# MarcoMeter/endless-memory-gym

Hardware: AMD Instinct MI355X
Metric: env steps/sec (aggregate) (higher is better)
Workload: dtype u8; 1 GPU; MortarMayhem-Grid-v0, 65536 envs/GPU x 1 GPU, 84x84x3 obs (u8_xyc), same-step auto-reset, uniform random actions generated on device; env_id=MortarMayhem-Grid-v0, envs_per_gpu=65536, envs_total=65536, parallelism=env-sharded x1, no data-path collective

## Files before the change

### endless-memory-gym_amd/csrc/mg_mortar.hip

```cpp
#include <memory>

#include "mg_atlas_v1.hpp"
#include "mg_lab.hpp"
#include "mg_option_sets.hpp"
#include "mg_stamps.hpp"
#include "mg_mortar_types.hpp"
#include "mg_mortar_compose.hpp"
#include "mg_raster_gather_v1.hpp"
#include "mg_mortar_step.hpp"
#include "mg_mortar_one_launch.hpp"
#include "mg_mortar_expert.hpp"
#include "mg_mortar_advance.hpp"
#include "mg_mortar_play.hpp"
#include "mg_mortar_trace.hpp"
#include "mg_mortar_next.hpp"

namespace mg {
using namespace v1;

__global__ __launch_bounds__(256) void mortar_init_kernel(int n, MortarState* state) {
    int i = blockIdx.x * blockDim.x + threadIdx.x;
    if (i >= n) return;
    MortarState s;
    memset(&s, 0, sizeof(s));
    s.disp_sprite = 0xFF;
    state[i] = s;
}

__global__ __launch_bounds__(256) void mortar_gt64_kernel(int n, const MortarState* state, double* out) {
    const int i = blockIdx.x * blockDim.x + threadIdx.x;
    if (i >= n) return;
    const MortarState s = state[i];
    out[2 * i] = s.tx / 5.0;
    out[2 * i + 1] = s.ty / 5.0;
}

__global__ __launch_bounds__(256) void mortar_gt64_masked_kernel(int n, const MortarState* state, double* out, const uint8_t* __restrict__ only) {
    const int i = blockIdx.x * blockDim.x + threadIdx.x;
    if (i >= n || !only[i]) return;
    const MortarState s = state[i];
    out[2 * i] = s.tx / 5.0;
    out[2 * i + 1] = s.ty / 5.0;
}

__global__ __launch_bounds__(256) void mortar_debug_desc_kernel(MortarParams P0, int n, MortarIO io, MortarDesc* out) {
    const int i = blockIdx.x * blockDim.x + threadIdx.x;
    if (i >= n) return;
    const MortarParams& P = io.set_of ? io.sets[set_index(io.set_of, i)] : P0;
    const MortarState s = io.state[i];
    const uint8_t* cmds = io.cmds + (size_t)i * P.cmd_cap;
    MortarDesc d = io.desc[i];
    {
        const bool have = s.disp_sprite != 0xFF;
        const int cx = (have && !s.disp_is_agent) ? s.disp_x : s.ax, cy = (have && !s.disp_is_agent) ? s.disp_y : s.ay;
        d.sx = (int16_t)(cx - P.sprite_dim / 2);
        d.sy = (int16_t)(cy - P.sprite_dim / 2);
        d.sprite = have ? s.disp_sprite : (uint8_t)0;
        d.tmpl = (uint16_t)((s.tiles_on && P.visual_feedback) ? 1 + s.tx * P.N + s.ty : 0);
        d.glyph_x0 = (int16_t)P.glyph_x0;
    }
    d.glyph = 0xFF;
    if (s.vis_pos < s.vis_len) {
        const int idx = (int)s.dbg_pops, period = s.show_dur + s.show_delay;
        io.state[i].dbg_pops = s.dbg_pops + 1;
        if (idx >= 0 && idx < (int)s.vis_len && period > 0) {
            const int k = idx / period, w = idx % period;
            d.glyph = (w < s.show_dur) ? cmds[s.vis_base + k] : (uint8_t)9;
        }
    }
    const int r = P.tile / 2;
    d.ring_x = (int16_t)(P.arena_x0 + P.tile * s.tx + P.tile / 2 - r);
    d.ring_y = (int16_t)(P.arena_x0 + P.tile * s.ty + P.tile / 2 - r);
    d.ring_on = 1;
    out[i] = d;
}

__device__ __forceinline__ MortarDesc mortar_debug_desc_one(const MortarParams& P, const MortarIO& io, int i) {
    const MortarState s = io.state[i];
    const uint8_t* cmds = io.cmds + (size_t)i * P.cmd_cap;
    MortarDesc d = io.desc[i];
    {
        const bool have = s.disp_sprite != 0xFF;
        const int cx = (have && !s.disp_is_agent) ? s.disp_x : s.ax, cy = (have && !s.disp_is_agent) ? s.disp_y : s.ay;
        d.sx = (int16_t)(cx - P.sprite_dim / 2);
        d.sy = (int16_t)(cy - P.sprite_dim / 2);
        d.sprite = have ? s.disp_sprite : (uint8_t)0;
        d.tmpl = (uint16_t)((s.tiles_on && P.visual_feedback) ? 1 + s.tx * P.N + s.ty : 0);
        d.glyph_x0 = (int16_t)P.glyph_x0;
    }
    d.glyph = 0xFF;
    if (s.vis_pos < s.vis_len) {
        const int idx = (int)s.dbg_pops, period = s.show_dur + s.show_delay;
        io.state[i].dbg_pops = s.dbg_pops + 1;
        if (idx >= 0 && idx < (int)s.vis_len && period > 0) {
            const int k = idx / period, w = idx % period;
            d.glyph = (w < s.show_dur) ? cmds[s.vis_base + k] : (uint8_t)9;
        }
    }
    const int r = P.tile / 2;
    d.ring_x = (int16_t)(P.arena_x0 + P.tile * s.tx + P.tile / 2 - r);
    d.ring_y = (int16_t)(P.arena_x0 + P.tile * s.ty + P.tile / 2 - r);
    d.ring_on = 1;
    return d;
}
__global__ __launch_bounds__(256) void mortar_debug_desc_picked_kernel(MortarParams P0, int n, MortarIO io, const int32_t* __restrict__ idx, int count,
                                                                       MortarDesc* rec) {
    const int j = blockIdx.x * blockDim.x + threadIdx.x;
    if (j >= count) return;
    const int i = idx ? idx[j] : j;
    if (i < 0) return;
    if (i >= n) return raise_error(io.err, ERR_FRAME_INDEX);
    const MortarParams& P = io.set_of ? io.sets[set_index(io.set_of, i)] : P0;
    rec[j] = mortar_debug_desc_one(P, io, i);
}

static const double SCALE = 0.25;

class MortarFamily : public Family {
   public:
    MortarFamily(int variant_id, int n) : Family(n), P_(sets_[0].P) {
        memset(&P_, 0, sizeof(P_));
        const int variant = variant_id >= 3 ? variant_id - 3 : variant_id;
        P_.variant = variant;
        P_.taskb = variant_id >= 3;
        agent_scale_ = 1.0 * SCALE;
        agent_speed_ = 12.0 * SCALE;
        P_.N = variant == V_ENDLESS ? 6 : 5;
        P_.allowed = variant == V_GRID ? 5 : 9;
        P_.visual_feedback = 1;
        P_.max_steps = -1;
        P_.initial_count = 1;
        P_.cmd_cap = variant == V_ENDLESS ? 512 : 32;
        if (variant == V_ENDLESS) {
            const int cap = lab_int("MEMGYM_EMM_CMD_CAP", 0);
            if (cap >= 4 && cap <= 512) P_.cmd_cap = cap;
        }
        MortarOpt& O = sets_[0];
        O.st_command_count.set(P_.command_count, {10});
        O.st_show_dur.set(P_.show_dur, {3});
        O.st_show_delay.set(P_.show_delay, {1});
        O.st_expl_dur.set(P_.expl_dur, {variant == V_GRID ? 2 : 6});
        O.st_expl_delay.set(P_.expl_delay, {variant == V_GRID ? 6 : 18});
        P_.r_fail = 0.0;
        P_.r_succ = 0.1;
        P_.r_ep_succ = 0.0;
        P_.r_new = 0.0;
        state_.alloc(n);
        cmds_.alloc((size_t)n * P_.cmd_cap);
        desc_.alloc(n);
        tdesc_.alloc(n);
        rng_.alloc(n);
        err_.alloc();
        claims_.alloc((size_t)((n + 255) / 256) * 4);
        handover_.alloc(n);
        rescues_.alloc(1);
        sets_.alloc();
        launch(mortar_init_kernel, dim3((n + 255) / 256), dim3(256), 0, 0, n, state_.p);
        MG_HIP(hipDeviceSynchronize());
        rebuild();
        sets_.defaults = P_;
    }

    void set_capacity(const std::string& what, int64_t v) override {
        if (!(P_.variant == V_ENDLESS && what == "commands")) return Family::set_capacity(what, v);
        if (v < 4 || v > 32768) throw OptionError{-3, "commands: 4 .. 32,768"};
        if (seeded_) throw std::runtime_error("mg_set_capacity: before the first reset");
        if (2 * P_.initial_count > v) throw OptionError{-3, "commands: below twice the initial_command_count in force"};
        MG_HIP(hipDeviceSynchronize());
        P_.cmd_cap = (int)v;
        cmds_.alloc((size_t)n_ * P_.cmd_cap);
        ++geom_gen_;
        sets_.refresh_geometry();
    }
    int64_t capacity(const std::string& what) const override {
        if (P_.variant == V_ENDLESS && what == "commands") return P_.cmd_cap;
        return Family::capacity(what);
    }
    void want_done_flag(uint32_t* flag_dev, uint32_t ticket) override {
        flag_dev_ = flag_dev;
        flag_ticket_ = ticket;
    }
    bool done_flag_stored() override {
        const bool stored = flag_stored_;
        flag_stored_ = false;
        return stored;
    }
    int action_dim() const override { return P_.variant == V_GRID ? 1 : 2; }
    int gt_dim() const override { return P_.variant == V_ENDLESS ? 2 : 0; }
    int vec_dim() const override { return P_.taskb ? VEC_DIM : 0; }
    void bind_vector_obs(float* dev) override {
        if (dev != vec_) ++geom_gen_;
        vec_ = dev;
    }
    const char* info_name(int k) const override {
        if (P_.variant == V_ENDLESS) return k == 0 ? "commands_completed" : (k == 1 ? "max_command_sequence" : nullptr);
        return k == 0 ? "success" : (k == 1 ? "commands_completed" : nullptr);
    }

    void set_option(const std::string& key, const double* v, int n) override { set_option_set(0, key, v, n); }
    void set_option_set(int set, const std::string& key, const double* v, int n) override {
        MortarOpt& O = sets_.ensure(set);
        MortarParams& P = O.P;
        const bool endless = P_.variant == V_ENDLESS;
        const OptionArg A{set, key, v, n, dirty_};
        if (key == "agent_scale") A.geometry(agent_scale_, v[0]);
        else if (key == "allowed_commands") {
            int a = A.integer();
            if (a < 4 || a > 9) throw OptionError{-4, "assert 4 <= allowed_commands <= 9"};
            P.allowed = a;
        }
        else if (!P_.taskb && key == "command_show_duration") O.st_show_dur.set(P.show_dur, A.int_list(1, 65535));
        else if (!P_.taskb && key == "command_show_delay") O.st_show_delay.set(P.show_delay, A.int_list(0, 65535));
        else if (key == "explosion_duration") O.st_expl_dur.set(P.expl_dur, A.int_list(1, 65535));
        else if (key == "explosion_delay") O.st_expl_delay.set(P.expl_delay, A.int_list(1, 65535));
        else if (key == "visual_feedback") P.visual_feedback = A.flag();
        else if (key == "reward_command_failure") P.r_fail = v[0];
        else if (key == "reward_command_success") P.r_succ = v[0];
        else if (endless && key == "max_steps") P.max_steps = A.integer();
        else if (endless && key == "initial_command_count") {
            int c = A.integer();
            if (c < 1 || c > P_.cmd_cap / 2) throw OptionError{-3, "initial_command_count out of the supported range"};
            P.initial_count = c;
        }
        else if (endless && key == "reward_new_command_success") P.r_new = v[0];
        else if (!endless && key == "arena_size") {
            int a = A.integer();
            if (a < 2 || a > MORTAR_MAX_N) throw OptionError{-4, "assert 2 <= arena_size <= 6"};
            if (a != P_.N) A.geometry(P_.N, a);
        }
        else if (!endless && key == "command_count") O.st_command_count.set(P.command_count, A.int_list(1, P_.taskb ? VEC_DIM / 9 : P_.cmd_cap));
        else if (!endless && key == "reward_episode_success") P.r_ep_succ = v[0];
        else if (P_.variant != V_GRID && key == "agent_speed") A.geometry(agent_speed_, v[0]);
        else throw OptionError{-2, "unknown reset parameter " + key};
    }
    void bind_option_sets(const int32_t* set_of_dev) override { sets_.bind(set_of_dev); }

    void reset(const int64_t* seeds, const uint8_t* mask, void* obs, float* gt, hipStream_t s) override {
        if (dirty_) rebuild();
        require_seeded(seeds);
        check_schedules();
        if (seeds) seeded_ = true;
        sets_.upload(s);
        with_bool(sets_.per_set(), [&](auto PS) {
            launch(mortar_reset_kernel<decltype(PS)::value>, dim3((n_ + 255) / 256), dim3(256), 0, s, P_, n_, io(), seeds, mask, gt_dim() ? gt : nullptr);
        });
        reset_frames(mask, [&](const uint8_t* m) { launch_raster_sparse<MortarComposer>(desc_.p, atlas_->dev(), obs, obs_format, n_, s, m); },
                     [&] { raster(obs, s); });
    }

    void step(const int32_t* actions, const uint8_t* active, void* obs, float* reward, uint8_t* done, float* gt, const mg_info_dev* info,
              int autoreset, hipStream_t s, void* final_frames) override {
        struct Consume {
            uint32_t*& flag;
            ~Consume() { flag = nullptr; }
        } consume{flag_dev_};
        flag_stored_ = false;
        const mg_info_dev ib = begin_step(info);
        sets_.upload(s);
        const MortarStepArgs sa = step_args(actions, reward, done, gt, ib, autoreset);
        if (obs && !active && one_launch(s)) {
            epoch_ = epoch_ % 255u + 1u;
            ++ticket_;
            const int logic_wgs = (n_ + 255) / 256;
            const int frames = frames_grid(n_);
            static const bool logic_last = lab_flag("MEMGYM_LAB_LOGIC_LAST", false);
            const bool store_flag = flag_dev_ && n_ == 1 && gt_dim() == 0 && obs_format == MG_OBS_U8_XYC;
            auto launch_step = [&](auto kernel, const MortarStepArgs& a, uint32_t* flag, uint32_t flag_ticket) {
                launch(kernel, dim3(logic_wgs + frames), dim3(256), RASTER_LDS, s, a, logic_wgs, logic_last ? frames : 0, epoch_, ticket_,
                               claims_.p, rescues_.p, atlas_->dev(), obs, flag, flag_ticket);
            };
            prof.begin(1, s);
            if (store_flag) {
                launch_step(mortar_step_raster_kernel<true>, sa, flag_dev_, flag_ticket_);
            } else if (ib.final_obs_dev && autoreset) {
                MortarStepArgs fa = sa;
                fa.tdesc = tdesc_.p;
                with_obs_format(obs_format, [&](auto F) { launch_step(mortar_step_raster_kernel<false, true, decltype(F)::value>, fa, nullptr, 0u); });
            } else {
                with_obs_format(obs_format, [&](auto F) { launch_step(mortar_step_raster_kernel<false, false, decltype(F)::value>, sa, nullptr, 0u); });
            }
            check_launch();
            ++one_launch_steps_;
            flag_stored_ = store_flag;
            prof.end(1, s);
            return;
        }
        prof.begin(0, s);
        const int sb = step_block(256);
        with_bool(sets_.per_set(), [&](auto PS) {
            if (final_frames) {
                with_bool(active != nullptr, [&](auto MASKED) {
                    launch(mortar_step_records_kernel<decltype(PS)::value, decltype(MASKED)::value>, dim3((n_ + sb - 1) / sb), dim3(sb), 0, s, sa, active,
                           (MortarDesc*)final_frames);
                });
            } else if (active) launch(mortar_step_masked_kernel<decltype(PS)::value>, dim3((n_ + sb - 1) / sb), dim3(sb), 0, s, sa, active);
            else launch(mortar_step_kernel<decltype(PS)::value>, dim3((n_ + sb - 1) / sb), dim3(sb), 0, s, sa);
        });
        end_logic(s);
        if (!obs) return;
        if (active) return masked_frames(obs, active, s);
        prof.begin(1, s);
        raster(obs, s);
        prof.end(1, s);
    }

    bool step_next(const int32_t* actions, const uint8_t* restart, uint8_t* restart_copy, void* obs, float* reward, uint8_t* done, float* gt,
                   const mg_info_dev* info, hipStream_t s) override {
        if (!lab_flag("MEMGYM_NEXT_FUSE", true)) return false;
        const mg_info_dev ib = begin_step(info);
        check_schedules();
        sets_.upload(s);
        const MortarStepArgs sa = step_args(actions, reward, done, gt, ib, 0);
        const int sb = step_block(256);
        prof.begin(0, s);
        with_bool(sets_.per_set(), [&](auto PS) {
            launch(mortar_step_next_kernel<decltype(PS)::value>, dim3((n_ + sb - 1) / sb), dim3(sb), 0, s, sa, restart, restart_copy);
        });
        end_logic(s);
        prof.begin(1, s);
        raster(obs, s);
        prof.end(1, s);
        with_bool(sets_.per_set(), [&](auto PS) {
            launch_checked(mortar_next_settle_kernel<decltype(PS)::value>, dim3((n_ + 255) / 256), dim3(256), 0, s, P_, n_, io(), (const uint8_t*)restart_copy);
        });
        return true;
    }

    bool advance(const AdvanceArgs& v, hipStream_t s) override {
        if (!lab_flag("MEMGYM_MORTAR_ADVANCE_FUSE", true)) return false;
        require_geometry();
        sets_.upload(s);
        const MortarStepArgs sa = step_args(v.actions, v.reward, v.done, v.gt, v.info, 1);
        rollout_chunks(v.steps, [&](int t0, int k) {
            with_bool(sets_.per_set(), [&](auto PS) {
                launch_checked(mortar_advance_kernel<decltype(PS)::value>, dim3((n_ + 255) / 256), dim3(256), 0, s, sa, advance_chunk(v, t0, k));
            });
        });
        return true;
    }
    bool play(const PlayArgs& v, hipStream_t s) override {
        if (!lab_flag("MEMGYM_MORTAR_PLAY_FUSE", true)) return false;
        require_geometry();
        sets_.upload(s);
        rollout_chunks(v.steps, [&](int t0, int k) {
            with_bool(sets_.per_set(), [&](auto PS) {
                launch_checked(mortar_play_kernel<decltype(PS)::value>, dim3((n_ + 255) / 256), dim3(256), 0, s, play_step_args(v, t0), play_chunk(v, t0, k));
            });
        });
        return true;
    }
    bool advance_traced(const AdvanceArgs& v, const TraceRows& tr, hipStream_t s) override {
        if (!lab_flag("MEMGYM_MORTAR_ADVANCE_FUSE", true)) return false;
        require_geometry();
        sets_.upload(s);
        const MortarStepArgs sa = step_args(v.actions, v.reward, v.done, v.gt, v.info, 1);
        const size_t row = (size_t)n_ * (size_t)action_dim();
        rollout_chunks(v.steps, [&](int t0, int k) {
            const MortarTraceRows rows{row_at((MortarDesc*)tr.frames, t0, n_), row_at(tr.actions, t0, row), row_at(tr.labels, t0, row), row_at(tr.reward, t0, n_),
                                       row_at(tr.done, t0, n_)};
            with_bool(sets_.per_set(), [&](auto PS) {
                launch_checked(mortar_advance_traced_kernel<decltype(PS)::value>, dim3((n_ + 255) / 256), dim3(256), 0, s, sa, advance_chunk(v, t0, k), rows);
            });
        });
        return true;
    }
    bool play_traced(const PlayArgs& v, void* frames, hipStream_t s) override {
        if (!lab_flag("MEMGYM_MORTAR_PLAY_FUSE", true)) return false;
        require_geometry();
        sets_.upload(s);
        rollout_chunks(v.steps, [&](int t0, int k) {
            with_bool(sets_.per_set(), [&](auto PS) {
                launch_checked(mortar_play_traced_kernel<decltype(PS)::value>, dim3((n_ + 255) / 256), dim3(256), 0, s, play_step_args(v, t0), play_chunk(v, t0, k),
                               row_at((MortarDesc*)frames, t0, n_));
            });
        });
        return true;
    }

    std::vector<std::pair<void*, size_t>> state_blobs() override {
        std::vector<std::pair<void*, size_t>> v = {{state_.p, state_.bytes()}, {cmds_.p, cmds_.bytes()}};
        rng_.blobs(v);
        return v;
    }

    std::vector<std::pair<void*, size_t>> instance_rows() override {
        std::vector<std::pair<void*, size_t>> v = {{state_.p, sizeof(MortarState)}, {cmds_.p, (size_t)P_.cmd_cap}, {desc_.p, sizeof(MortarDesc)}};
        rng_.rows(v);
        if (vec_) v.push_back({vec_, sizeof(float) * VEC_DIM});
        return v;
    }

    void expert_actions(const ExpertArgs& x, hipStream_t s) override {
        require_geometry();
        sets_.upload(s);
        launch_checked(mortar_expert_kernel, expert_grid(n_), dim3(EXPERT_BLOCK), 0, s, P_, n_, io(), x);
    }
    void ground_truth64(double* out, hipStream_t s, const uint8_t* only = nullptr) override {
        if (!gt_dim() || !out) return;
        if (only) return launch_checked(mortar_gt64_masked_kernel, dim3((n_ + 255) / 256), dim3(256), 0, s, n_, state_.p, out, only);
        launch_checked(mortar_gt64_kernel, dim3((n_ + 255) / 256), dim3(256), 0, s, n_, state_.p, out);
    }
    bool debug_counter(const std::string& name, int64_t* out) override {
        if (name == "cmd_list_max" || name == "cmd_list_ge12") {
            std::vector<MortarState> h(n_);
            MG_HIP(hipDeviceSynchronize());
            MG_HIP(hipMemcpy(h.data(), state_.p, sizeof(MortarState) * (size_t)n_, hipMemcpyDeviceToHost));
            int64_t mx = 0, ge = 0;
            for (const MortarState& s : h) {
                mx = s.num_cmds > mx ? s.num_cmds : mx;
                ge += s.num_cmds >= 12;
            }
            *out = name == "cmd_list_max" ? mx : ge;
            return true;
        }
        if (name == "one_launch_steps") {
            *out = one_launch_steps_;
            return true;
        }
        if (name != "one_launch_rescues") return false;
        uint32_t v = 0;
        MG_HIP(hipMemcpy(&v, rescues_.p, sizeof v, hipMemcpyDeviceToHost));
        *out = (int64_t)v;
        return true;
    }

    void raster_debug(void* frames, hipStream_t s) override {
        debug_frames<MortarDesc>(
            s, [&](MortarDesc* dbg) { launch(mortar_debug_desc_kernel, dim3((n_ + 255) / 256), dim3(256), 0, s, P_, n_, io(), dbg); },
            [&](MortarDesc* dbg) { launch_raster<MortarDebugComposer>(dbg, atlas_->dev(), frames, MG_OBS_U8_XYC, n_, s); });
    }

    void save_debug_records(const int32_t* idx, int count, void* rec, hipStream_t s) override {
        sets_.upload(s);
        launch_checked(mortar_debug_desc_picked_kernel, dim3((count + 255) / 256), dim3(256), 0, s, P_, n_, io(), idx, count, (MortarDesc*)rec);
    }
    void draw_debug_records(const void* records, int n_records, const int32_t* pick, int count, int size, void* rgb, hipStream_t s) override {
        launch_raster_debug_gather<MortarDebugComposer>((const MortarDesc*)records, atlas_->dev(), rgb, size, n_records, pick, count, err_.dev, s);
        check_launch();
    }

   private:
    uint32_t* flag_dev_ = nullptr;
    uint32_t flag_ticket_ = 0;
    bool flag_stored_ = false;
    int64_t one_launch_steps_ = 0;
    uint32_t ticket_ = 0;
    uint32_t epoch_ = 0;
    bool one_launch(hipStream_t s) { return fuse_step() && !sets_.per_set() && !stream_capturing(s); }
    static bool fuse_step() {
        static const bool on = lab_flag("MEMGYM_MORTAR_FUSE", true);
        return on;
    }
    void check_schedules() {
        for (size_t k = 0; k < sets_.size(); ++k) {
            const MortarOpt& O = sets_[k];
            const long long n_max = P_.variant == V_ENDLESS ? O.P.initial_count : O.st_command_count.max(O.P.command_count);
            if (!P_.taskb && n_max * ((long long)O.st_show_dur.max(O.P.show_dur) + O.st_show_delay.max(O.P.show_delay)) > 65535)
                throw OptionError{-3, "command_count x (command_show_duration + command_show_delay) exceeds the 65,535 entries of this build's display schedule"};
        }
    }
    MortarStepArgs step_args(const int32_t* actions, float* reward, uint8_t* done, float* gt, const mg_info_dev& ib, int autoreset) {
        return MortarStepArgs{P_, n_, io(), actions, reward, done, gt_dim() ? gt : nullptr, ib, autoreset, handover_.p, nullptr};
    }
    template <class F>
    static void rollout_chunks(int steps, F&& f) {
        for (int t0 = 0; t0 < steps; t0 += ADVANCE_MAX_STEPS) f(t0, steps - t0 < ADVANCE_MAX_STEPS ? steps - t0 : ADVANCE_MAX_STEPS);
    }
    template <class T>
    static T* row_at(T* base, int t0, size_t width) {
        return base ? base + (size_t)t0 * width : nullptr;
    }
    static MortarAdvanceArgs advance_chunk(const AdvanceArgs& v, int t0, int k) {
        return MortarAdvanceArgs{k, t0 == 0 ? 1 : 0, v.eps, v.seed, v.step0 + (uint64_t)t0, v.actions, v.out};
    }
    MortarStepArgs play_step_args(const PlayArgs& v, int t0) {
        return step_args(row_at(v.tape, t0, (size_t)n_ * (size_t)action_dim()), v.reward, v.done, v.gt, v.info, v.episode ? 0 : 1);
    }
    MortarPlayArgs play_chunk(const PlayArgs& v, int t0, int k) const {
        return MortarPlayArgs{k, t0 == 0 ? 1 : 0, t0 + k == v.steps ? 1 : 0, v.episode, n_ * action_dim(), v.active, v.alive, row_at(v.reward_trace, t0, n_),
                              row_at(v.done_trace, t0, n_), v.played, v.out};
    }
    MortarIO io() {
        MortarIO o;
        o.state = state_.p;
        o.cmds = cmds_.p;
        o.rng = rng_.view();
        o.desc = desc_.p;
        o.vec = vec_;
        o.err = err_.dev;
        o.sets = sets_.dev();
        o.set_of = sets_.set_of();
        return o;
    }

    void rebuild() {
        int radius = 0;
        std::vector<Stamp> sprites = build_agent_sprites(P_.variant == V_GRID ? 1.0 * SCALE : agent_scale_, &radius);
        std::vector<Stamp> glyphs = build_glyphs(SCALE);
        P_.tile = (int)(56 * SCALE);
        P_.arena_x0 = SCREEN / 2 - ((P_.tile * P_.N) >> 1);
        P_.radius = radius;
        P_.sprite_dim = sprites[0].w;
        double inv = 1.0 / std::sqrt(2.0);
        P_.v_axis = (1.0 / 1.0) * agent_speed_;
        P_.v_diag = inv * agent_speed_;
        P_.v_axis_i = (int)P_.v_axis;
        P_.v_diag_i = (int)P_.v_diag;
        P_.off_lo = (int)(-8 * SCALE);
        P_.off_hi = (int)(8 * SCALE);

        atlas_.reset(new Atlas());
        for (auto& sp : sprites) atlas_->add_stamp(sp);
        for (auto& g : glyphs) atlas_->add_stamp(g);
        {
            const int r = P_.tile / 2;
            Stamp ring_stamp(2 * r, 2 * r);
            circle(ring_stamp, r, r, r, (int)(8 * SCALE), 6);
            atlas_->add_stamp(ring_stamp);
        }
        atlas_->set_templates(build_mortar_templates(P_.N, SCALE, SCREEN));
        atlas_->upload();
        P_.glyph_x0 = (int)((SCREEN / 2) - std::floor(88 * SCALE / 2));
        dirty_ = false;
        ++geom_gen_;
        sets_.refresh_geometry();
    }

    struct MortarOpt {
        MortarParams P;
        OptListStore st_command_count, st_show_dur, st_show_delay, st_expl_dur, st_expl_delay;
        static void copy_geometry(MortarParams& d, const MortarParams& s) {
            d.variant = s.variant; d.N = s.N; d.taskb = s.taskb; d.cmd_cap = s.cmd_cap; d.arena_x0 = s.arena_x0; d.tile = s.tile;
            d.radius = s.radius; d.sprite_dim = s.sprite_dim; d.glyph_x0 = s.glyph_x0; d.v_axis_i = s.v_axis_i; d.v_diag_i = s.v_diag_i;
            d.off_lo = s.off_lo; d.off_hi = s.off_hi; d.v_axis = s.v_axis; d.v_diag = s.v_diag;
        }
    };

    void raster_only(void* obs, const uint8_t* only, hipStream_t s) override {
        launch_raster<MortarComposer>(desc_.p, atlas_->dev(), obs, obs_format, n_, s, only);
        check_launch();
    }
    std::pair<const void*, size_t> frame_rows() override { return {desc_.p, sizeof(MortarDesc)}; }
    void draw_records(const void* records, int n_records, const int32_t* pick, int count, int fmt, void* obs, hipStream_t s) override {
        launch_raster_gather<MortarComposer, false>((const MortarDesc*)records, atlas_->dev(), obs, fmt, n_records, pick, count, err_.dev, s);
        check_launch();
    }
    void draw_records_padded(const void* records, int n_records, const int32_t* pick, int count, int fmt, void* obs, hipStream_t s) override {
        launch_raster_gather<MortarComposer, true>((const MortarDesc*)records, atlas_->dev(), obs, fmt, n_records, pick, count, err_.dev, s);
        check_launch();
    }
    bool keeps_final_obs(hipStream_t s) override {
        static const bool wanted = lab_flag("MEMGYM_MORTAR_FINAL_FUSED", true);
        return wanted && one_launch(s);
    }

    void raster(void* obs, hipStream_t s) { raster_only(obs, nullptr, s); }

    OptionSets<MortarOpt> sets_;
    MortarParams& P_;
    std::unique_ptr<Atlas> atlas_;
    double agent_scale_, agent_speed_;
    float* vec_ = nullptr;
    DevArray<MortarState> state_;
    DevArray<uint8_t> cmds_;
    DevArray<MortarDesc> desc_;
    DevArray<uint32_t> claims_, rescues_;
    DevArray<uint64_t> handover_, tdesc_;
};

Family* make_mortar(int variant, int num_envs) { return new MortarFamily(variant, num_envs); }

}

#ifdef MG_LAB
extern "C" int mg_lab_set_window_offsets(const long long* off, int n) {
    long long v[16] = {0};
    for (int i = 0; i < n && i < 16; ++i) v[i] = off[i];
    return hipMemcpyToSymbol(HIP_SYMBOL(mg::v1::g_lab_win_off), v, sizeof v) == hipSuccess ? 0 : -1;
}
#endif
```

### endless-memory-gym_amd/csrc/mg_mortar_one_launch.hpp

```cpp
#pragma once
#include "mg_mortar_compose.hpp"
#include "mg_mortar_step.hpp"

namespace mg {
using namespace v1;

constexpr unsigned long long RESCUE_AFTER_TICKS = 20000;
__device__ __forceinline__ MortarDesc desc_from_handover(uint32_t lo, uint32_t hi, int glyph_x0) {
    const Handover f = unpack_handover(lo, hi);
    MortarDesc d;
    d.sx = (int16_t)f.sx, d.sy = (int16_t)f.sy, d.tmpl = (uint16_t)f.tmpl, d.sprite = (uint8_t)f.sprite, d.glyph = (uint8_t)f.glyph;
    d.glyph_x0 = (int16_t)glyph_x0;
    d.ring_x = d.ring_y = 0, d.ring_on = (uint8_t)f.ring_on, d.reserved = 0;
    return d;
}
constexpr int one_launch_wgs_per_cu(int fmt) { return fmt == MG_OBS_U8_XYC || fmt == MG_OBS_U8_CYX ? 7 : 6; }
template <bool DONE_FLAG, bool FINAL = false, int FMT = MG_OBS_U8_XYC>
__global__ __launch_bounds__(256, one_launch_wgs_per_cu(FMT)) void mortar_step_raster_kernel(MortarStepArgs a, int logic_wgs, int logic_base, uint32_t epoch,
                                                                    uint32_t ticket, uint32_t* claims, uint32_t* rescues,
                                                                    RasterAtlas A, void* __restrict__ obs, uint32_t* done_flag, uint32_t done_ticket) {
    constexpr bool ONE_BYTE = one_launch_wgs_per_cu(FMT) == 7;
    auto store = [](uint8_t* frame, void* dst, int env, int t) {
        if constexpr (ONE_BYTE) store_frame<FMT, false>(frame, dst, env, t);
        else store_frame<FMT, false, false, 1>(frame, dst, env, t & 255);
    };
    const int n = a.n;
    const int tid = threadIdx.x, lane = tid & 63;
    const int rel = (int)blockIdx.x - logic_base;
    const bool is_logic = rel >= 0 && rel < logic_wgs;
    auto claim = [&](int q) -> bool {
        uint32_t old = 0;
        if (lane == 0) old = __hip_atomic_exchange(claims + q, ticket, __ATOMIC_RELAXED, __HIP_MEMORY_SCOPE_AGENT);
        return (uint32_t)__builtin_amdgcn_readfirstlane((int)old) != ticket;
    };
    if (is_logic) {
        const int q = rel * 4 + (tid >> 6), i = q * 64 + lane;
#if defined(MG_LABV) && MG_LABV >= 1
        if (i < n) mortar_step_body<true, false, false, FINAL, DONE_FLAG>(i, a, epoch);
#else
        if (i < n) mortar_step_body<true, true, false, FINAL, DONE_FLAG>(i, a, epoch, claims + q, ticket);
#endif
        return;
    }
    extern __shared__ __attribute__((aligned(16))) uint8_t smem[];
    RasterCtx R = make_ctx(smem, A);
    const int stride = (int)gridDim.x - logic_wgs;
    for (int v = (int)blockIdx.x < logic_base ? (int)blockIdx.x : (int)blockIdx.x - logic_wgs; v < n; v += stride) {
        const int env = xcd_grouped_frame(v, n);
        const uint64_t* src = a.handover + env;
        uint32_t lo, hi;
        bool tried = false;
        unsigned long long t0 = 0;
        for (int polls = 0;; ++polls) {
            const uint64_t w = __hip_atomic_load(src, __ATOMIC_RELAXED, __HIP_MEMORY_SCOPE_AGENT);
            lo = (uint32_t)__builtin_amdgcn_readfirstlane((int)(uint32_t)w);
            hi = (uint32_t)__builtin_amdgcn_readfirstlane((int)(uint32_t)(w >> 32));
            if ((hi >> (HANDOVER_EPOCH_SHIFT - 32)) == epoch) break;
#if defined(MG_LABV) && MG_LABV >= 2
            if (false) {
#else
            if (polls == 0) t0 = wall_clock64();
            if (!tried && (polls & 15) == 15 && wall_clock64() - t0 >= RESCUE_AFTER_TICKS) {
#endif
                tried = true;
                if (claim(env >> 6)) {
                    const MortarStepArgs MG_KERNARG_AS* ka = kernarg_reread<MortarStepArgs>();
                    int i = (env >> 6) * 64 + lane;
                    asm volatile("" : "+v"(i));
                    if (i < n) mortar_step_body<true, false, false, FINAL, DONE_FLAG>(i, *(const MortarStepArgs*)ka, epoch);
                    if (lane == 0) atomicAdd(rescues, 1u);
                    continue;
                }
            }
            __builtin_amdgcn_s_sleep(4);
        }
        const MortarDesc d = desc_from_handover(lo, hi, a.P.glyph_x0);
        if constexpr (FINAL) {
            if (d.ring_on) {
                const MortarStepArgs MG_KERNARG_AS* ka = kernarg_reread<MortarStepArgs>();
                const uint64_t tw = __hip_atomic_load(ka->tdesc + env, __ATOMIC_RELAXED, __HIP_MEMORY_SCOPE_AGENT);
                const MortarDesc td = desc_from_handover((uint32_t)__builtin_amdgcn_readfirstlane((int)(uint32_t)tw), (uint32_t)__builtin_amdgcn_readfirstlane((int)(uint32_t)(tw >> 32)), a.P.glyph_x0);
                int tt = tid;
                asm volatile("" : "+v"(tt));
                R.tid = tt;
                MortarComposer::compose(&td, R);
                __syncthreads();
                store(smem, ka->info.final_obs_dev, env, tt);
                __syncthreads();
            }
        }
        if (MortarComposer::skip(&d)) continue;
        int t = tid;
        asm volatile("" : "+v"(t));
        R.tid = t;
        MortarComposer::compose(&d, R);
        __syncthreads();
        store(smem, obs, env, t);
        __syncthreads();
    }
    if constexpr (DONE_FLAG) {
        __builtin_amdgcn_fence(__ATOMIC_RELEASE, "");
        __syncthreads();
        if (tid == 0) __hip_atomic_store(done_flag, done_ticket, __ATOMIC_RELAXED, __HIP_MEMORY_SCOPE_SYSTEM);
    }
}
}
```

### endless-memory-gym_amd/csrc/mg_mortar_step.hpp

```cpp
#pragma once
#include "mg_mortar_types.hpp"

namespace mg {
constexpr uint32_t pack_deltas(const int (&v)[9]) {
    uint32_t m = 0;
    for (int c = 0; c < 9; ++c) m |= (uint32_t)(v[c] + 1) << (2 * c);
    return m;
}
constexpr int kDxHost[9] = {1, 0, -1, 0, 0, 1, 1, -1, -1}, kDyHost[9] = {0, 1, 0, -1, 0, 1, -1, 1, -1};
constexpr uint32_t CMD_DX_BITS = pack_deltas(kDxHost), CMD_DY_BITS = pack_deltas(kDyHost);
__device__ __forceinline__ int cmd_dx(int c) { return (int)((CMD_DX_BITS >> (2 * c)) & 3u) - 1; }
__device__ __forceinline__ int cmd_dy(int c) { return (int)((CMD_DY_BITS >> (2 * c)) & 3u) - 1; }

__device__ __forceinline__ int floordiv(int a, int b) {
    int q = a / b;
    return (a % b != 0 && a < 0) ? q - 1 : q;
}
__device__ __forceinline__ int mod6(int a) { return ((a % 6) + 6) % 6; }
__device__ __forceinline__ int round_haz(double v) { return v >= 0 ? (int)floor(v + 0.5) : -(int)floor(-v + 0.5); }

__constant__ int8_t kCmdOneHot[9] = {1, 4, 2, 3, 0, 5, 6, 7, 8};
constexpr int VEC_DIM = 180;

__device__ void mortar_reset(const MortarParams& P, MortarState& s, Pcg& g, uint8_t* cmds, MortarDesc& d, float* gt, float* vec) {
    if (s.disp_sprite != 0xFF && s.disp_is_agent) {
        s.disp_x = s.ax;
        s.disp_y = s.ay;
        s.disp_is_agent = 0;
    }
    int half = P.tile / 2;
    int tile_id = g.integers(0, P.N * P.N);
    int cx = P.arena_x0 + P.tile * (tile_id / P.N) + half;
    int cy = P.arena_x0 + P.tile * (tile_id % P.N) + half;
    if (P.variant == V_ENDLESS || (P.taskb && P.variant == V_FREE)) {
        cx += g.integers(P.off_lo, P.off_hi);
        cy += g.integers(P.off_lo, P.off_hi);
    }
    s.ax = (int16_t)cx;
    s.ay = (int16_t)cy;
    s.rot8 = 0;
    int nx = floordiv(cx - P.arena_x0, P.tile), ny = floordiv(cy - P.arena_x0, P.tile);
    s.nx = (int8_t)nx;
    s.ny = (int8_t)ny;
    s.gx = (uint8_t)nx;
    s.gy = (uint8_t)ny;

    int n;
    if (P.variant == V_ENDLESS) {
        n = P.initial_count;
        for (int i = 0; i < n; ++i) cmds[i] = (uint8_t)g.integers(0, P.allowed);
    } else {
        n = choice(g, P.command_count);
        int px = nx, py = ny;
        for (int i = 0; i < n; ++i) {
            uint32_t valid = 0;
#pragma unroll
            for (int c = 0; c < 9; ++c) {
                const int qx = px + cmd_dx(c), qy = py + cmd_dy(c);
                if (c < P.allowed && qx >= 0 && qx < P.N && qy >= 0 && qy < P.N) valid |= 1u << c;
            }
            const int pick = g.integers(0, __popc(valid));
            uint32_t m = valid;
            for (int k = 0; k < pick; ++k) m &= m - 1;
            const int c = __ffs(m) - 1;
            cmds[i] = (uint8_t)c;
            px += cmd_dx(c);
            py += cmd_dy(c);
        }
    }
    s.num_cmds = (uint16_t)n;
    if (P.taskb) {
        s.show_dur = s.show_delay = 0;
    } else {
        s.show_dur = (uint16_t)choice(g, P.show_dur);
        s.show_delay = (uint16_t)choice(g, P.show_delay);
    }
    s.vis_len = (uint16_t)(n * (s.show_dur + s.show_delay));
    s.vis_base = 0;
    s.vis_pos = 1;
    s.dbg_pops = 0;
    int first = cmds[0];
    uint8_t glyph = s.show_dur > 0 ? (uint8_t)first : (uint8_t)9;
    if (P.variant == V_ENDLESS) {
        s.tx = (int8_t)mod6(nx + cmd_dx(first));
        s.ty = (int8_t)mod6(ny + cmd_dy(first));
    } else {
        s.tx = (int8_t)(nx + cmd_dx(first));
        s.ty = (int8_t)(ny + cmd_dy(first));
    }
    s.cur_cmd = 0;
    s.cmd_steps = 0;
    s.verify_step = 0;
    s.total_completed = 0;
    s.tiles_on = 0;
    s.t = 0;
    s.ep_len = 0;
    s.ep_sum = 0.0;
    s.expl_dur = (uint16_t)choice(g, P.expl_dur);
    s.expl_delay = (uint16_t)choice(g, P.expl_delay);

    d.tmpl = 0;
    d.sprite = 0;
    d.sx = (int16_t)(cx - P.sprite_dim / 2);
    d.sy = (int16_t)(cy - P.sprite_dim / 2);
    d.glyph = glyph;
    if (gt) {
        gt[0] = (float)(s.tx / 5.0);
        gt[1] = (float)(s.ty / 5.0);
    }
    if (vec) {
        for (int k = 0; k < VEC_DIM; ++k) vec[k] = 0.0f;
        for (int c = 0; c < n && c < VEC_DIM / 9; ++c) vec[9 * c + kCmdOneHot[cmds[c]]] = 1.0f;
    }
}

template <bool PS>
__global__ __launch_bounds__(256) void mortar_reset_kernel(MortarParams P0, int n, MortarIO io, const int64_t* seeds,
                                                           const uint8_t* mask, float* gt) {
    int i = blockIdx.x * blockDim.x + threadIdx.x;
    if (i >= n) return;
    const MortarParams& P = PS ? io.sets[set_index(io.set_of, i)] : P0;
    MortarDesc d;
    memset(&d, 0, sizeof(d));
    d.glyph_x0 = (int16_t)P.glyph_x0;
    if (mask && !mask[i]) {
        d.tmpl = 0xFFFF;
        io.desc[i] = d;
        return;
    }
    Pcg g;
    if (seeds) g.seed((uint64_t)seeds[i]);
    else g.load(io.rng, i);
    MortarState s = io.state[i];
    mortar_reset(P, s, g, io.cmds + (size_t)i * P.cmd_cap, d, gt ? gt + 2 * i : nullptr, io.vec ? io.vec + (size_t)i * VEC_DIM : nullptr);
    io.state[i] = s;
    g.store(io.rng, i);
    io.desc[i] = d;
}

template <bool FUSED, bool CLAIM = false, bool PS = false, bool FINAL = false, bool ORDERED = false, bool RECORDS = false>
__device__ __forceinline__ void mortar_step_body(int i, const MortarStepArgs& a, uint32_t epoch, uint32_t* claim_word = nullptr,
                                                 uint32_t ticket = 0u, const int32_t* actions_row = nullptr, MortarDesc* final_frames = nullptr) {
    uint32_t claimed_by = 0u;
    if constexpr (CLAIM) {
        claimed_by = ticket + 1u;
        if ((threadIdx.x & 63) == 0) claimed_by = __hip_atomic_exchange(claim_word, ticket, __ATOMIC_RELAXED, __HIP_MEMORY_SCOPE_AGENT);
    }
    const MortarIO& io = a.io;
    const MortarParams& P = PS ? io.sets[set_index(io.set_of, i)] : a.P;
    const int32_t* const actions = actions_row ? actions_row : a.actions;
    float* const reward_out = a.reward_out;
    uint8_t* const done_out = a.done_out;
    float* const gt = a.gt;
    const mg_info_dev& info = a.info;
    const int autoreset = a.autoreset;
    const bool one_action = P.variant == V_GRID;
    int act0 = actions[one_action ? i : 2 * i], act1 = actions[one_action ? i : 2 * i + 1];
    Pcg g;
    bool rng_loaded = !FUSED;
    if constexpr (!FUSED) g.load(io.rng, i);
    MortarState s = io.state[i];
    asm volatile("" : "+v"(act0), "+v"(act1));
    if constexpr (!FUSED) g.pin();
    if constexpr (CLAIM) {
        asm volatile("" : "+v"(claimed_by));
        if ((uint32_t)__builtin_amdgcn_readfirstlane((int)claimed_by) == ticket) return;
    }
    uint8_t* cmds = io.cmds + (size_t)i * P.cmd_cap;
    double reward = 0.0;
    bool done = false, cap = false;
    int success = 0;
    uint8_t glyph = 0xFF;
    bool rng_used = false;

    if (s.vis_pos < s.vis_len) {
        int period = s.show_dur + s.show_delay;
        int k = s.vis_pos / period, w = s.vis_pos % period;
        glyph = (w < s.show_dur) ? cmds[s.vis_base + k] : (uint8_t)9;
        s.vis_pos++;
        if (P.variant != V_ENDLESS || s.disp_sprite == 0xFF) {
            s.disp_sprite = 0;
            s.disp_is_agent = 1;
        }
    } else {
        int ax = s.ax, ay = s.ay;
        if (P.variant == V_GRID) {
            int a = act0;
            int rot = s.rot8 * 45;
            if (a == 1) rot = (rot + 90) % 360;
            if (a == 2) rot = (rot + 270) % 360;
            int gx = s.gx, gy = s.gy;
            if (a == 3) {
                int face = rot / 90;
                if (face == 0) { if (gy > 0) gy--; }
                else if (face == 3) { if (gx < P.N - 1) gx++; }
                else if (face == 2) { if (gy < P.N - 1) gy++; }
                else { if (gx > 0) gx--; }
                ax = P.arena_x0 + P.tile * gx + P.tile / 2;
                ay = P.arena_x0 + P.tile * gy + P.tile / 2;
            }
            s.gx = (uint8_t)gx;
            s.gy = (uint8_t)gy;
            s.rot8 = (uint8_t)(rot / 45);
        } else {
            int a0 = act0, a1 = act1;
            int dxs = a0 == 1 ? -1 : (a0 == 2 ? 1 : 0), dys = a1 == 1 ? -1 : (a1 == 2 ? 1 : 0);
            int rot = s.rot8 * 45;
            if (a0 == 1) rot = 90;
            if (a0 == 2) rot = 270;
            if (a1 == 1) rot = 0;
            if (a1 == 2) rot = 180;
            if (dxs < 0 && dys < 0) rot = 45;
            if (dxs < 0 && dys > 0) rot = 135;
            if (dxs > 0 && dys < 0) rot = 315;
            if (dxs > 0 && dys > 0) rot = 225;
            s.rot8 = (uint8_t)(rot / 45);
            bool diag = dxs != 0 && dys != 0;
            if (P.variant == V_FREE) {
                int v = diag ? P.v_diag_i : P.v_axis_i;
                ax += dxs * v;
                ay += dys * v;
                int lo = P.arena_x0 + P.radius, hi = P.arena_x0 + P.tile * P.N - P.radius;
                ax = ax > hi ? hi : ax;
                ax = ax < lo ? lo : ax;
                ay = ay > hi ? hi : ay;
                ay = ay < lo ? lo : ay;
            } else {
                double v = diag ? P.v_diag : P.v_axis;
                ax = round_haz((double)ax + dxs * v);
                ay = round_haz((double)ay + dys * v);
                double left = P.arena_x0, right = P.arena_x0 + P.tile * P.N, off = P.radius * 0.5;
                double x = ax, y = ay;
                if (x > right + off) x = left - off;
                if (x < left - off) x = right + off;
                if (y > right + off) y = left - off;
                if (y < left - off) y = right + off;
                ax = round_haz(x);
                ay = round_haz(y);
            }
        }
        s.ax = (int16_t)ax;
        s.ay = (int16_t)ay;
        s.disp_sprite = s.rot8;
        s.disp_is_agent = 1;
        int nx = floordiv(ax - P.arena_x0, P.tile), ny = floordiv(ay - P.arena_x0, P.tile);
        s.nx = (int8_t)nx;
        s.ny = (int8_t)ny;
        bool on_target = (nx == s.tx) && (ny == s.ty);

        bool verify = (s.cmd_steps % s.expl_delay == 0) && s.cmd_steps > 0;
        if (verify && !s.tiles_on) {
            if (s.cur_cmd < s.num_cmds) {
                s.cur_cmd++;
                s.tiles_on = 1;
                if (on_target) {
                    reward += P.r_succ;
                    if (P.variant == V_ENDLESS) {
                        s.total_completed++;
                        if (s.cur_cmd == s.num_cmds) reward += P.r_new;
                    }
                } else {
                    done = true;
                    reward += P.r_fail;
                }
            }
            if (s.cur_cmd >= s.num_cmds) {
                if (P.variant == V_ENDLESS) {
                    if (!rng_loaded) g.load(io.rng, i);
                    rng_loaded = true;
                    rng_used = true;
                    int nc = g.integers(0, P.allowed);
                    if (s.num_cmds < P.cmd_cap) {
                        cmds[s.num_cmds] = (uint8_t)nc;
                        s.vis_base = s.num_cmds;
                        s.num_cmds++;
                    } else {
                        raise_error(io.err, ERR_CMD_OVERFLOW);
                        done = true;
                        cap = true;
                        s.vis_base = (uint16_t)(s.num_cmds - 1);
                    }
                    s.cur_cmd = 0;
                    s.verify_step = 0;
                    s.vis_pos = 0;
                    s.vis_len = (uint16_t)(s.show_dur + s.show_delay);
                    s.dbg_pops = 0;
                } else {
                    done = true;
                    success = 1;
                    reward += P.r_ep_succ;
                }
            }
            s.cmd_steps = 1;
        }
        if (s.tiles_on) {
            if (s.verify_step % s.expl_dur == 0 && s.verify_step > 0) {
                s.tiles_on = 0;
                s.verify_step = 0;
                if (s.cur_cmd < s.num_cmds) {
                    int c = cmds[s.cur_cmd];
                    if (P.variant == V_ENDLESS) {
                        s.tx = (int8_t)mod6(s.tx + cmd_dx(c));
                        s.ty = (int8_t)mod6(s.ty + cmd_dy(c));
                    } else {
                        s.tx = (int8_t)(s.tx + cmd_dx(c));
                        s.ty = (int8_t)(s.ty + cmd_dy(c));
                    }
                }
            } else {
                if (!on_target) {
                    done = true;
                    reward = P.r_fail;
                }
                s.verify_step++;
            }
        } else {
            s.cmd_steps++;
        }
    }

    if (P.variant == V_ENDLESS) {
        s.t++;
        if (s.t == P.max_steps) done = true;
    }
    s.ep_sum += reward;
    s.ep_len++;

    if (done) {
        if (info.ep_reward_dev) info.ep_reward_dev[i] = s.ep_sum;
        if (info.ep_length_dev) info.ep_length_dev[i] = s.ep_len;
        if (P.variant == V_ENDLESS) {
            if (info.aux_dev[0]) info.aux_dev[0][i] = (float)s.total_completed;
            if (info.aux_dev[1]) info.aux_dev[1][i] = (float)(s.num_cmds > 1 ? s.num_cmds - 1 : 0);
        } else {
            if (info.aux_dev[0]) info.aux_dev[0][i] = (float)success;
            if (info.aux_dev[1]) info.aux_dev[1][i] = (float)((double)((int)s.cur_cmd - 1 + success) / (double)s.num_cmds);
        }
    }
    reward_out[i] = (float)reward;
    if (info.reward64_dev) info.reward64_dev[i] = reward;
    done_out[i] = done ? 1 : 0;
    if (info.capacity_dev) info.capacity_dev[i] = cap ? 1 : 0;

    MortarDesc d;
    memset(&d, 0, sizeof(d));
    d.glyph_x0 = (int16_t)P.glyph_x0;
    if constexpr (RECORDS) {
        if (done) {
            MortarDesc td = d;
            const int tcx = s.disp_is_agent ? s.ax : s.disp_x, tcy = s.disp_is_agent ? s.ay : s.disp_y;
            td.sx = (int16_t)(tcx - P.sprite_dim / 2);
            td.sy = (int16_t)(tcy - P.sprite_dim / 2);
            td.sprite = s.disp_sprite;
            td.glyph = glyph;
            td.tmpl = (uint16_t)((s.tiles_on && P.visual_feedback) ? 1 + s.tx * P.N + s.ty : 0);
            final_frames[i] = td;
        }
    }
    if (done && autoreset) {
        if constexpr (FINAL) {
            const int tcx = s.disp_is_agent ? s.ax : s.disp_x, tcy = s.disp_is_agent ? s.ay : s.disp_y;
            const uint64_t tw = pack_handover(tcx - P.sprite_dim / 2, tcy - P.sprite_dim / 2, (s.tiles_on && P.visual_feedback) ? 1 + s.tx * P.N + s.ty : 0,
                                              0, s.disp_sprite, glyph, 0);
            __hip_atomic_store(a.tdesc + i, tw, __ATOMIC_RELAXED, __HIP_MEMORY_SCOPE_AGENT);
        }
        if (!rng_loaded) g.load(io.rng, i);
        rng_loaded = true;
        rng_used = true;
        mortar_reset(P, s, g, cmds, d, (gt && P.variant == V_ENDLESS) ? gt + 2 * i : nullptr, io.vec ? io.vec + (size_t)i * VEC_DIM : nullptr);
        if constexpr (FINAL) d.ring_on = 1;
    } else {
        int cx = s.disp_is_agent ? s.ax : s.disp_x, cy = s.disp_is_agent ? s.ay : s.disp_y;
        d.sx = (int16_t)(cx - P.sprite_dim / 2);
        d.sy = (int16_t)(cy - P.sprite_dim / 2);
        d.sprite = s.disp_sprite;
        d.glyph = glyph;
        d.tmpl = (uint16_t)((s.tiles_on && P.visual_feedback) ? 1 + s.tx * P.N + s.ty : 0);
        if (gt && P.variant == V_ENDLESS) {
            gt[2 * i] = (float)(s.tx / 5.0);
            gt[2 * i + 1] = (float)(s.ty / 5.0);
        }
    }
    if constexpr (FUSED) {
        if constexpr (FINAL || ORDERED) asm volatile("s_waitcnt vmcnt(0)" ::: "memory");
        __hip_atomic_store(a.handover + i, pack_handover(d.sx, d.sy, d.tmpl, d.ring_on, d.sprite, d.glyph, epoch), __ATOMIC_RELAXED, __HIP_MEMORY_SCOPE_AGENT);
    }
    if (rng_used) g.store(io.rng, i);
    io.state[i] = s;
    io.desc[i] = d;
}

template <bool PS>
__global__ __launch_bounds__(256) void mortar_step_kernel(MortarStepArgs a) {
    const int i = blockIdx.x * blockDim.x + threadIdx.x;
    if (i < a.n) mortar_step_body<false, false, PS>(i, a, 0u);
}

template <bool PS>
__global__ __launch_bounds__(256) void mortar_step_masked_kernel(MortarStepArgs a, const uint8_t* __restrict__ active) {
    const int i = blockIdx.x * blockDim.x + threadIdx.x;
    if (i >= a.n) return;
    if (active[i]) mortar_step_body<false, false, PS>(i, a, 0u);
    else masked_out(i, a.reward_out, a.done_out, a.info);
}

template <bool PS, bool MASKED>
__global__ __launch_bounds__(256) void mortar_step_records_kernel(MortarStepArgs a, const uint8_t* __restrict__ active, MortarDesc* __restrict__ final_frames) {
    const int i = blockIdx.x * blockDim.x + threadIdx.x;
    if (i >= a.n) return;
    if (!MASKED || active[i]) mortar_step_body<false, false, PS, false, false, true>(i, a, 0u, nullptr, 0u, nullptr, final_frames);
    else masked_out(i, a.reward_out, a.done_out, a.info);
}
}
```

Baseline: 297.3 million env steps/s.

## Publish handover word early for non-reset envs and prefetch command row

In the fused one-launch step, envs that do not reset now build their render descriptor and publish the handover word right after the logic finishes, before the reset path and the state/rng/desc writebacks. The goal is to let raster workgroups that are polling the handover start composing sooner. The first 16 bytes of each env's command row are loaded up front alongside the state, so the glyph lookup avoids a dependent global load. Optional wall-clock instrumentation is added behind a lab define, and the CYX format keeps the late publish.

```diff
diff --git a/endless-memory-gym_amd/csrc/mg_mortar.hip b/endless-memory-gym_amd/csrc/mg_mortar.hip
--- a/endless-memory-gym_amd/csrc/mg_mortar.hip
+++ b/endless-memory-gym_amd/csrc/mg_mortar.hip
@@ -579,3 +579,14 @@
     return hipMemcpyToSymbol(HIP_SYMBOL(mg::v1::g_lab_win_off), v, sizeof v) == hipSuccess ? 0 : -1;
 }
 #endif
+
+#ifdef MG_LAB_MORTAR_CLOCK
+extern "C" int mg_lab_mortar_clock(unsigned long long* host, int n_words, int clear) {
+    if (clear) {
+        void* p = nullptr;
+        if (hipGetSymbolAddress(&p, HIP_SYMBOL(mg::g_lab_mortar_clock)) != hipSuccess) return -1;
+        return hipMemset(p, 0, sizeof(mg::g_lab_mortar_clock)) == hipSuccess ? 0 : -1;
+    }
+    return hipMemcpyFromSymbol(host, HIP_SYMBOL(mg::g_lab_mortar_clock), sizeof(unsigned long long) * (size_t)n_words) == hipSuccess ? 0 : -1;
+}
+#endif
diff --git a/endless-memory-gym_amd/csrc/mg_mortar_one_launch.hpp b/endless-memory-gym_amd/csrc/mg_mortar_one_launch.hpp
--- a/endless-memory-gym_amd/csrc/mg_mortar_one_launch.hpp
+++ b/endless-memory-gym_amd/csrc/mg_mortar_one_launch.hpp
@@ -20,6 +20,7 @@
                                                                     uint32_t ticket, uint32_t* claims, uint32_t* rescues,
                                                                     RasterAtlas A, void* __restrict__ obs, uint32_t* done_flag, uint32_t done_ticket) {
     constexpr bool ONE_BYTE = one_launch_wgs_per_cu(FMT) == 7;
+    constexpr bool LATE_WORD = FMT == MG_OBS_U8_CYX;
     auto store = [](uint8_t* frame, void* dst, int env, int t) {
         if constexpr (ONE_BYTE) store_frame<FMT, false>(frame, dst, env, t);
         else store_frame<FMT, false, false, 1>(frame, dst, env, t & 255);
@@ -36,9 +37,9 @@
     if (is_logic) {
         const int q = rel * 4 + (tid >> 6), i = q * 64 + lane;
 #if defined(MG_LABV) && MG_LABV >= 1
-        if (i < n) mortar_step_body<true, false, false, FINAL, DONE_FLAG>(i, a, epoch);
+        if (i < n) mortar_step_body<true, false, false, FINAL, DONE_FLAG, false, LATE_WORD>(i, a, epoch);
 #else
-        if (i < n) mortar_step_body<true, true, false, FINAL, DONE_FLAG>(i, a, epoch, claims + q, ticket);
+        if (i < n) mortar_step_body<true, true, false, FINAL, DONE_FLAG, false, LATE_WORD>(i, a, epoch, claims + q, ticket);
 #endif
         return;
     }
@@ -48,6 +49,8 @@
     for (int v = (int)blockIdx.x < logic_base ? (int)blockIdx.x : (int)blockIdx.x - logic_wgs; v < n; v += stride) {
         const int env = xcd_grouped_frame(v, n);
         const uint64_t* src = a.handover + env;
+        [[maybe_unused]] const int clock_row = v < stride ? MORTAR_CLOCK_ROW_OF_FRAME(v) : -1;
+        if (tid == 0) MORTAR_CLOCK(clock_row, 0);
         uint32_t lo, hi;
         bool tried = false;
         unsigned long long t0 = 0;
@@ -67,13 +70,14 @@
                     const MortarStepArgs MG_KERNARG_AS* ka = kernarg_reread<MortarStepArgs>();
                     int i = (env >> 6) * 64 + lane;
                     asm volatile("" : "+v"(i));
-                    if (i < n) mortar_step_body<true, false, false, FINAL, DONE_FLAG>(i, *(const MortarStepArgs*)ka, epoch);
+                    if (i < n) mortar_step_body<true, false, false, FINAL, DONE_FLAG, false, LATE_WORD>(i, *(const MortarStepArgs*)ka, epoch);
                     if (lane == 0) atomicAdd(rescues, 1u);
                     continue;
                 }
             }
             __builtin_amdgcn_s_sleep(4);
         }
+        if (tid == 0) MORTAR_CLOCK(clock_row, 1);
         const MortarDesc d = desc_from_handover(lo, hi, a.P.glyph_x0);
         if constexpr (FINAL) {
             if (d.ring_on) {
@@ -96,6 +100,7 @@
         MortarComposer::compose(&d, R);
         __syncthreads();
         store(smem, obs, env, t);
+        if (tid == 0) MORTAR_CLOCK(clock_row, 2);
         __syncthreads();
     }
     if constexpr (DONE_FLAG) {
diff --git a/endless-memory-gym_amd/csrc/mg_mortar_step.hpp b/endless-memory-gym_amd/csrc/mg_mortar_step.hpp
--- a/endless-memory-gym_amd/csrc/mg_mortar_step.hpp
+++ b/endless-memory-gym_amd/csrc/mg_mortar_step.hpp
@@ -138,9 +138,43 @@
     io.desc[i] = d;
 }
 
-template <bool FUSED, bool CLAIM = false, bool PS = false, bool FINAL = false, bool ORDERED = false, bool RECORDS = false>
+constexpr bool mortar_early_word(bool fused, bool ordered) {
+#ifdef MG_LAB_MORTAR_NO_EARLY
+    return false;
+#else
+    return fused && !ordered;
+#endif
+}
+constexpr bool mortar_row_prefetch(bool fused) {
+#ifdef MG_LAB_MORTAR_NO_ROW
+    return false;
+#else
+    return fused;
+#endif
+}
+constexpr int CMD_ROW_PREFETCH = 16;
+
+#ifdef MG_LAB_MORTAR_CLOCK
+constexpr int MORTAR_CLOCK_STEP_ROWS = 4096, MORTAR_CLOCK_FRAME_ROWS = 16384, MORTAR_CLOCK_COLS = 8;
+static __device__ unsigned long long g_lab_mortar_clock[(MORTAR_CLOCK_STEP_ROWS + MORTAR_CLOCK_FRAME_ROWS) * MORTAR_CLOCK_COLS];
+#define MORTAR_CLOCK(row, col) do { if ((row) >= 0 && (row) < MORTAR_CLOCK_STEP_ROWS + MORTAR_CLOCK_FRAME_ROWS) atomicMax(&g_lab_mortar_clock[(row) * MORTAR_CLOCK_COLS + (col)], (unsigned long long)wall_clock64()); } while (0)
+#define MORTAR_CLOCK_AFTER(row, col, ...) do { asm volatile("" ::__VA_ARGS__); MORTAR_CLOCK(row, col); } while (0)
+#define MORTAR_CLOCK_FLAG(row, col) do { if ((row) >= 0 && (row) < MORTAR_CLOCK_STEP_ROWS) atomicMax(&g_lab_mortar_clock[(row) * MORTAR_CLOCK_COLS + (col)], 1ull); } while (0)
+#define MORTAR_CLOCK_ROW_OF_FRAME(v) (MORTAR_CLOCK_STEP_ROWS + (v))
+#define MORTAR_CLOCK_ROW_OF_STEP(i) (((i) >> 6) < MORTAR_CLOCK_STEP_ROWS ? (i) >> 6 : -1)
+#else
+#define MORTAR_CLOCK_ROW_OF_FRAME(v) (-1)
+#define MORTAR_CLOCK_ROW_OF_STEP(i) (-1)
+#define MORTAR_CLOCK(row, col) ((void)0)
+#define MORTAR_CLOCK_AFTER(row, col, ...) ((void)0)
+#define MORTAR_CLOCK_FLAG(row, col) ((void)0)
+#endif
+
+template <bool FUSED, bool CLAIM = false, bool PS = false, bool FINAL = false, bool ORDERED = false, bool RECORDS = false, bool LATE_WORD = false>
 __device__ __forceinline__ void mortar_step_body(int i, const MortarStepArgs& a, uint32_t epoch, uint32_t* claim_word = nullptr,
                                                  uint32_t ticket = 0u, const int32_t* actions_row = nullptr, MortarDesc* final_frames = nullptr) {
+    [[maybe_unused]] const int clock_row = FUSED ? MORTAR_CLOCK_ROW_OF_STEP(i) : -1;
+    MORTAR_CLOCK(clock_row, 0);
     uint32_t claimed_by = 0u;
     if constexpr (CLAIM) {
         claimed_by = ticket + 1u;
@@ -159,6 +193,14 @@
     Pcg g;
     bool rng_loaded = !FUSED;
     if constexpr (!FUSED) g.load(io.rng, i);
+    constexpr bool EARLY = mortar_early_word(FUSED, ORDERED) && !LATE_WORD, ROW = mortar_row_prefetch(FUSED);
+    uint32_t row[CMD_ROW_PREFETCH / 4] = {0u, 0u, 0u, 0u};
+    bool row_in = false;
+    if constexpr (ROW) {
+        row_in = P.cmd_cap >= CMD_ROW_PREFETCH;
+        const uint8_t* const from = row_in ? io.cmds + (size_t)i * P.cmd_cap : (const uint8_t*)(io.state + i);
+        __builtin_memcpy(row, from, CMD_ROW_PREFETCH);
+    }
     MortarState s = io.state[i];
     asm volatile("" : "+v"(act0), "+v"(act1));
     if constexpr (!FUSED) g.pin();
@@ -166,6 +208,7 @@
         asm volatile("" : "+v"(claimed_by));
         if ((uint32_t)__builtin_amdgcn_readfirstlane((int)claimed_by) == ticket) return;
     }
+    MORTAR_CLOCK_AFTER(clock_row, 1, "v"((int)s.vis_pos), "v"((int)s.ep_len));
     uint8_t* cmds = io.cmds + (size_t)i * P.cmd_cap;
     double reward = 0.0;
     bool done = false, cap = false;
@@ -176,7 +219,18 @@
     if (s.vis_pos < s.vis_len) {
         int period = s.show_dur + s.show_delay;
         int k = s.vis_pos / period, w = s.vis_pos % period;
-        glyph = (w < s.show_dur) ? cmds[s.vis_base + k] : (uint8_t)9;
+        if constexpr (ROW) {
+            const int at = s.vis_base + k;
+            if (w >= s.show_dur) glyph = (uint8_t)9;
+            else if (row_in && at < CMD_ROW_PREFETCH) {
+                const uint32_t lo = (at & 4) ? row[1] : row[0], hi = (at & 4) ? row[3] : row[2];
+                glyph = (uint8_t)(((at & 8) ? hi : lo) >> (8 * (at & 3)));
+            } else {
+                glyph = cmds[at];
+            }
+        } else {
+            glyph = (w < s.show_dur) ? cmds[s.vis_base + k] : (uint8_t)9;
+        }
         s.vis_pos++;
         if (P.variant != V_ENDLESS || s.disp_sprite == 0xFF) {
             s.disp_sprite = 0;
@@ -357,7 +411,24 @@
             final_frames[i] = td;
         }
     }
+    auto publish = [&]() {
+        __hip_atomic_store(a.handover + i, pack_handover(d.sx, d.sy, d.tmpl, d.ring_on, d.sprite, d.glyph, epoch), __ATOMIC_RELAXED, __HIP_MEMORY_SCOPE_AGENT);
+    };
+    const bool resets = done && autoreset;
+    if constexpr (EARLY) {
+        if (!resets) {
+            int cx = s.disp_is_agent ? s.ax : s.disp_x, cy = s.disp_is_agent ? s.ay : s.disp_y;
+            d.sx = (int16_t)(cx - P.sprite_dim / 2);
+            d.sy = (int16_t)(cy - P.sprite_dim / 2);
+            d.sprite = s.disp_sprite;
+            d.glyph = glyph;
+            d.tmpl = (uint16_t)((s.tiles_on && P.visual_feedback) ? 1 + s.tx * P.N + s.ty : 0);
+            publish();
+            MORTAR_CLOCK(clock_row, 2);
+        }
+    }
     if (done && autoreset) {
+        MORTAR_CLOCK_FLAG(clock_row, 5);
         if constexpr (FINAL) {
             const int tcx = s.disp_is_agent ? s.ax : s.disp_x, tcy = s.disp_is_agent ? s.ay : s.disp_y;
             const uint64_t tw = pack_handover(tcx - P.sprite_dim / 2, tcy - P.sprite_dim / 2, (s.tiles_on && P.visual_feedback) ? 1 + s.tx * P.N + s.ty : 0,
@@ -370,24 +441,36 @@
         mortar_reset(P, s, g, cmds, d, (gt && P.variant == V_ENDLESS) ? gt + 2 * i : nullptr, io.vec ? io.vec + (size_t)i * VEC_DIM : nullptr);
         if constexpr (FINAL) d.ring_on = 1;
     } else {
-        int cx = s.disp_is_agent ? s.ax : s.disp_x, cy = s.disp_is_agent ? s.ay : s.disp_y;
-        d.sx = (int16_t)(cx - P.sprite_dim / 2);
-        d.sy = (int16_t)(cy - P.sprite_dim / 2);
-        d.sprite = s.disp_sprite;
-        d.glyph = glyph;
-        d.tmpl = (uint16_t)((s.tiles_on && P.visual_feedback) ? 1 + s.tx * P.N + s.ty : 0);
+        if constexpr (!EARLY) {
+            int cx = s.disp_is_agent ? s.ax : s.disp_x, cy = s.disp_is_agent ? s.ay : s.disp_y;
+            d.sx = (int16_t)(cx - P.sprite_dim / 2);
+            d.sy = (int16_t)(cy - P.sprite_dim / 2);
+            d.sprite = s.disp_sprite;
+            d.glyph = glyph;
+            d.tmpl = (uint16_t)((s.tiles_on && P.visual_feedback) ? 1 + s.tx * P.N + s.ty : 0);
+        }
         if (gt && P.variant == V_ENDLESS) {
             gt[2 * i] = (float)(s.tx / 5.0);
             gt[2 * i + 1] = (float)(s.ty / 5.0);
         }
     }
     if constexpr (FUSED) {
-        if constexpr (FINAL || ORDERED) asm volatile("s_waitcnt vmcnt(0)" ::: "memory");
-        __hip_atomic_store(a.handover + i, pack_handover(d.sx, d.sy, d.tmpl, d.ring_on, d.sprite, d.glyph, epoch), __ATOMIC_RELAXED, __HIP_MEMORY_SCOPE_AGENT);
+        if constexpr (EARLY) {
+            if (resets) {
+                if constexpr (FINAL) asm volatile("s_waitcnt vmcnt(0)" ::: "memory");
+                publish();
+                MORTAR_CLOCK(clock_row, 3);
+            }
+        } else {
+            if constexpr (FINAL || ORDERED) asm volatile("s_waitcnt vmcnt(0)" ::: "memory");
+            publish();
+            MORTAR_CLOCK(clock_row, 3);
+        }
     }
     if (rng_used) g.store(io.rng, i);
     io.state[i] = s;
     io.desc[i] = d;
+    MORTAR_CLOCK(clock_row, 4);
 }
 
 template <bool PS>
```

Result: no change. 296.5 million env steps/s (-0.3%).
